# gpustack/llama-box

Measured on AMD Instinct MI355X. Metric: decode tokens/sec (batch-1) + prefill tok/s, Llama-3-8B Q4_K_M, higher is better.
Workload: dtype q4_K/q6_K weights x q8_K activations (int8 dot, f32 accumulate)

## Files before the change

llama_box_amd/csrc/backend.cpp:

```cpp
#include <dlfcn.h>

#include <algorithm>
#include <chrono>
#include <mutex>
#include <thread>

#include "common.h"
#include "kernels.h"

namespace mi355x {

int log_level() {
    static int lvl = [] {
        const char * e = getenv("GGML_MI355X_LOG");
        return e ? atoi(e) : 0;
    }();
    return lvl;
}

struct device_ctx {
    int device = 0;
    std::string name, description;
    ggml_backend_buffer_type buft{};
    ggml_backend_buffer_type buft_rowpar{};
// ... 163 lines not shown
        u->failed = true;
        return nullptr;
    }
    u->device = device;
    return u;
}
static void uploader_drain(int device) {
    if (device < 0 || device >= GGML_MI355X_MAX_DEVICES) return;
    uploader * u = &g_uploaders[device];
    if (u->device != device) return;
    std::lock_guard<std::mutex> lock(u->mtx);
    if (!u->in_flight) return;
    HIP_SOFT(hipStreamSynchronize(u->stream));
    for (bool & b : u->busy) b = false;
    u->in_flight = false;
}
static void uploader_join(int device, hipStream_t s) {
    if (device < 0 || device >= GGML_MI355X_MAX_DEVICES) return;
    uploader * u = &g_uploaders[device];
    if (u->device != device || !u->in_flight) return;
    std::lock_guard<std::mutex> lock(u->mtx);
    if (!u->in_flight) return;
    if (hipEventQuery(u->last) == hipSuccess) {
        for (bool & b : u->busy) b = false;
        u->in_flight = false;
        return;
    }
    (void) hipGetLastError();
    HIP_SOFT(hipStreamWaitEvent(s, u->last, 0));
}
// ... 255 lines not shown
static const char * be_get_name(ggml_backend_t be) { return ((backend_ctx *) be->context)->name.c_str(); }
static void be_free(ggml_backend_t be) {
    backend_ctx * c = (backend_ctx *) be->context;
    HIP_SOFT(hipSetDevice(c->device));
    HIP_SOFT(hipStreamSynchronize(c->stream));
    free_graph_cache(c);
    ip_free(c);
    tp_free(c);
    free_split_helpers(c);
    if (c->ws) HIP_NOTE(hipFree(c->ws));
    if (c->up_ring) HIP_NOTE(hipHostFree(c->up_ring));
    if (c->fa_lists) HIP_NOTE(hipFree(c->fa_lists));
    if (c->rope_tab) HIP_NOTE(hipFree(c->rope_tab));
    if (c->fa_arrive) HIP_NOTE(hipFree(c->fa_arrive));
    if (c->ss_buf) HIP_NOTE(hipFree(c->ss_buf));
    HIP_SOFT(hipStreamDestroy(c->stream));
    delete c;
    delete be;
}
void flush_uploads(backend_ctx * c) {
    if (c->up_pending.n == 0) return;
    launch_upload_multi(c->stream, c->up_pending);
    c->up_pending.n = 0;
}
static void be_set_tensor_async(ggml_backend_t be, ggml_tensor * t, const void * data, size_t offset, size_t size) {
    backend_ctx * c = (backend_ctx *) be->context;
    if (ip_any()) ip_host_access(t->view_src ? t->view_src->buffer : t->buffer, true);
    HIP_SOFT(hipSetDevice(c->device));
    note_mask_upload(t, data, offset, size);
    {
// ... 58 lines not shown
        HIP_SOFT(hipMemcpyAsync(dst->data, src->data, n, hipMemcpyDeviceToDevice, cs->stream));
    } else {
        HIP_SOFT(hipSetDevice(cs->device));
        HIP_SOFT(hipMemcpyPeerAsync(dst->data, cd->device, src->data, cs->device, n, cs->stream));
    }
    if (be_src != be_dst) {
        hipEvent_t ev;
        HIP_NOTE(hipEventCreateWithFlags(&ev, hipEventDisableTiming));
        HIP_SOFT(hipEventRecord(ev, cs->stream));
        HIP_SOFT(hipSetDevice(cd->device));
        HIP_SOFT(hipStreamWaitEvent(cd->stream, ev, 0));
        HIP_NOTE(hipEventDestroy(ev));
    }
    return true;
}
static void be_synchronize(ggml_backend_t be) {
    backend_ctx * c = (backend_ctx *) be->context;
    HIP_SOFT(hipSetDevice(c->device));
    flush_uploads(c);
    uploader_drain(c->device);
    HIP_SOFT(hipStreamSynchronize(c->stream));
}
static enum ggml_status be_graph_compute(ggml_backend_t be, ggml_cgraph * g) {
    backend_ctx * c = (backend_ctx *) be->context;
    if (hipSetDevice(c->device) != hipSuccess) return GGML_STATUS_FAILED;
    flush_uploads(c);
    uploader_join(c->device, c->stream);
    return graph_compute(c, g);
}
static void be_event_record(ggml_backend_t be, ggml_backend_event_t ev) {
    backend_ctx * c = (backend_ctx *) be->context;
    flush_uploads(c);
    HIP_SOFT(hipEventRecord((hipEvent_t) ev->context, c->stream));
}
static void be_event_wait(ggml_backend_t be, ggml_backend_event_t ev) {
// ... 180 lines not shown
    else if (k == "mmq_min_cols") c->opt.mmq_min_cols = v;
    else if (k == "mmq_i8") c->opt.mmq_i8 = v != 0;
    else if (k == "mm_merge") c->opt.mm_merge = v != 0;
    else if (k == "mmq_bn") c->opt.mmq_bn = v;
    else if (k == "mmq_skinny") c->opt.mmq_skinny = v != 0;
    else if (k == "skinny_rope") c->opt.skinny_rope = v != 0;
    else if (k == "skinny_mix") c->opt.skinny_mix = v != 0;
    else if (k == "softmax_mm") c->opt.softmax_mm = v != 0;
    else if (k == "attn_nf") c->opt.attn_nf = v != 0;
    else if (k == "fa_self_merge") c->opt.fa_self_merge = v != 0;
    else if (k == "ss_partials") c->opt.ss_partials = v != 0;
    else if (k == "tp_p2p") { if (!tp_p2p_enable(c, v != 0)) return -2; }
    else if (k == "tp_p2p_reset") { if (!tp_p2p_reset(c)) return -2; }
    else if (k == "fa_splits") c->opt.fa_splits = v;
    else if (k == "fa_wo") c->opt.fa_wo = v != 0;
    else if (k == "small_uploads") c->opt.small_uploads = v != 0;
    else if (k == "small_downloads") c->opt.small_downloads = v != 0;
    else if (k == "timing") c->opt.timing = v != 0;
    else if (k == "exec_update") c->opt.exec_update = v;
    else if (k == "shadow_capture") c->opt.shadow_capture = v;
    else if (k == "q80_min_cols") c->opt.q80_min_cols = v;
    else if (k == "decode_copy") c->opt.decode_copy = v != 0;
    else if (k == "decode_copy_headroom_gib") c->opt.decode_copy_headroom_gib = v;
    else if (k == "clear_failure") { if (v) clear_hip_failure(); }
    else if (k == "staged_upload") g_staged_upload.store(v != 0);
    else return -1;
    HIP_SOFT(hipStreamSynchronize(c->stream));
    free_graph_cache(c);
    return 0;
}
static int64_t api_get_stat(ggml_backend_t be, const char * key) {
    if (!be_is_ours(be)) return -1;
// ... 15 lines not shown
    if (k == "elided_conts") return c->st.elided_conts;
    if (k == "decode_copy_tensors") return c->st.decode_copy_tensors;
    if (k == "decode_copy_bytes") return c->st.decode_copy_bytes;
    if (k == "decode_copy_launches") return c->st.decode_copy_launches;
    if (k == "graph_exec_update_failures") return c->st.graph_exec_update_failures;
    if (k == "graph_evictions") return c->st.graph_evictions;
    if (k == "graph_cache_size") return (int64_t) c->graphs.size();
    if (k == "graph_launch_host_ns") return c->st.graph_launch_host_ns;
    if (k == "kernel_downloads") return c->st.kernel_downloads;
    if (k == "kv_image_nodes") return c->st.kv_image_nodes;
    if (k == "kv_native_nodes") return c->st.kv_native_nodes;
    if (k == "graph_key_host_ns") return c->st.graph_key_host_ns;
    if (k == "graph_compute_host_ns") return c->st.graph_compute_host_ns;
    if (k == "graph_key_fast_hits") return c->st.graph_key_fast_hits;
    if (k == "graph_key_collisions") return c->st.graph_key_collisions;
    if (k == "graph_early_captures") return c->st.graph_early_captures;
    if (k == "graph_shadow_captures") return c->st.graph_shadow_captures;
    if (k == "graph_capture_walk_ns") return c->st.graph_capture_walk_ns;
    if (k == "graph_exec_update_ns") return c->st.graph_exec_update_ns;
    if (k == "graph_shadow_eager_ns") return c->st.graph_shadow_eager_ns;
    if (k == "graph_exec_updates") return c->st.graph_exec_updates;
    if (k == "skinny_launches") return c->st.skinny_launches;
    if (k == "mmid_launches") return c->st.mmid_launches;
    if (k == "wide_launches") return c->st.wide_launches;
    if (k == "tiled_launches") return c->st.tiled_launches;
    if (k == "rope_epilogues") return c->st.rope_epilogues;
    if (k.rfind("ip_", 0) == 0) return ip_stat(c, key);
    if (k == "staged_upload_bytes") return (int64_t) g_uploaders[c->device].bytes;
    if (k == "staged_upload_us") return (int64_t) (g_uploaders[c->device].seconds * 1e6);
    return -1;
// ... 142 lines not shown
```

llama_box_amd/csrc/common.h:

```cpp
#pragma once
#include <hip/hip_runtime.h>
#include <hip/hip_ext.h>

#include <cstdint>
#include <cstdio>
#include <cstdlib>
#include <cstring>
#include <atomic>
#include <map>
#include <mutex>
#include <string>
#include <unordered_map>
#include <vector>

#include "../../include/ggml_mi355x.h"

#define MI_LOG(level, ...)                                    \
    do {                                                      \
        if ((level) <= mi355x::log_level()) {                 \
            fprintf(stderr, "ggml-mi355x: " __VA_ARGS__);     \
            fprintf(stderr, "\n");                            \
        }                                                     \
    } while (0)
#define MI_ERR(...) MI_LOG(0, __VA_ARGS__)
// ... 78 lines not shown
    bool qkv = true;
    int mmvq_max_cols = 2;
    int mmq_min_cols = 3;
    bool mmq_i8 = true;
    bool mm_merge = true;
    bool ss_partials = true;
    bool fa_self_merge = false;
    bool attn_nf = true;
    bool softmax_mm = true;
    bool skinny_rope = true;
    bool skinny_mix = true;
    bool mmq_skinny = true;
    int mmq_bn = 0;
    int fa_splits = 0;
    bool fa_wo = false;
    bool small_uploads = true;
    bool small_downloads = true;
    bool timing = false;
    int decode_copy_headroom_gib = 2;
    bool decode_copy = [] { const char * e = getenv("GGML_MI355X_DECODE_COPY"); return e ? atoi(e) != 0 : true; }();
    int exec_update = [] { const char * e = getenv("GGML_MI355X_EXEC_UPDATE"); return e ? atoi(e) : 1; }();
    int shadow_capture = [] { const char * e = getenv("GGML_MI355X_SHADOW_CAPTURE"); return e ? atoi(e) : 1; }();
    int q80_min_cols = [] { const char * e = getenv("GGML_MI355X_Q80_MIN_COLS"); return e ? atoi(e) : 33; }();
};

struct stats {
    int64_t graph_launches = 0, graph_captures = 0, eager_graphs = 0, kernel_launches = 0, fused_nodes = 0, allreduces = 0;
    int64_t p2p_allreduces = 0;
    int64_t ss_handoffs = 0;
    int64_t skinny_launches = 0;
    int64_t mmid_launches = 0;
    int64_t wide_launches = 0;
// ... 9 lines not shown
    int64_t kv_native_nodes = 0;
    int64_t kv_image_nodes = 0;
    int64_t kernel_downloads = 0;
    int64_t graph_early_captures = 0;
    int64_t graph_shadow_captures = 0;
    int64_t graph_capture_walk_ns = 0, graph_exec_update_ns = 0, graph_shadow_eager_ns = 0;
    int64_t graph_exec_updates = 0;
    int64_t decode_copy_tensors = 0;
    int64_t decode_copy_bytes = 0;
    int64_t decode_copy_launches = 0;
    int64_t elided_conts = 0;
    int64_t step_heads = 0;
    int64_t graph_exec_update_failures = 0;
    int64_t graph_evictions = 0;
    int64_t graph_key_collisions = 0;
};

struct tp_state;
struct split_helper;
struct ip_engine;

struct cached_graph {
    hipGraph_t graph = nullptr;
    hipGraphExec_t exec = nullptr;
    int seen = 0;
    uint64_t last_use = 0;
    int64_t allreduces = 0;
    int n_nodes = 0;
    int fa_form = 0;
    bool early_failed = false;
// ... 19 lines not shown
    uint64_t q8_epoch = 0;
    std::unordered_map<uint64_t, cached_graph> graphs;
    cached_graph * last_graph = nullptr;
    std::vector<uint64_t> key_scratch;
    uint64_t tick = 0;
    uint64_t decode_epoch = 0;
    bool capturing = false;
    bool mm_q5_major = false;
    tp_state * tp = nullptr;
    ip_engine * ip = nullptr;
    std::vector<split_helper *> split_helpers;
    hipEvent_t split_ready = nullptr;
    char * up_ring = nullptr;
    size_t up_cap = 0, up_head = 0;
    upload_batch up_pending{};
    double * ss_buf = nullptr;
    unsigned * fa_arrive = nullptr;
    static constexpr int fa_arrive_slots = 16384;
    float * rope_tab = nullptr;
    static constexpr int rope_tab_floats = 4096 * 256;
    int * fa_lists = nullptr;
    size_t fa_lists_bytes = 0;
    std::map<std::string, timing_slot> timing;
    std::vector<std::pair<std::string, std::pair<hipEvent_t, hipEvent_t>>> pending_events;
};

inline bool ensure_dyn_lds(const void * kernel, size_t bytes, std::atomic<uint32_t> & done) {
    int dev = 0;
    if (hipGetDevice(&dev) != hipSuccess || dev < 0 || dev >= 32) dev = 0;
    const uint32_t bit = 1u << dev;
// ... 98 lines not shown
```

llama_box_amd/csrc/graph.cpp:

```cpp
#include <algorithm>
#include <chrono>
#include <cmath>

#include "kernels.h"

namespace mi355x {

static bool is_kq23_type(int t) { return t == GGML_TYPE_Q2_K || t == GGML_TYPE_Q3_K; }
static bool is_quant(int t) { return t == GGML_TYPE_Q4_K || t == GGML_TYPE_Q5_K || t == GGML_TYPE_Q6_K || t == GGML_TYPE_Q8_0 || is_l32_type(t) || is_kq23_type(t); }
static bool l32_layout_ok(const ggml_tensor * a) {
    const size_t al = (a->type == GGML_TYPE_Q4_1 || a->type == GGML_TYPE_Q5_1 || a->type == GGML_TYPE_Q2_K) ? 4 : 2;
    if ((((uintptr_t) a->data) % al) || (a->nb[1] % al) || (a->nb[2] % al) || (a->nb[3] % al)) return false;
    return !buffer_is_rowpar(a->view_src ? a->view_src->buffer : a->buffer) && !buffer_is_split(a->buffer);
}
static inline int mmq_min_cols_for(const backend_ctx * c, int wtype) {
    if (is_kq23_type(wtype)) return 9;
    if (c->opt.mmq_min_cols != 3) return c->opt.mmq_min_cols;
    return (wtype == GGML_TYPE_Q4_K || (wtype == GGML_TYPE_Q6_K && !c->mm_q5_major)) ? 2 : 3;
}
static int act_kind(int wtype) {
    if (wtype == GGML_TYPE_Q4_1 || wtype == GGML_TYPE_Q5_1) return GGML_TYPE_Q8_1;
    return (wtype == GGML_TYPE_Q8_0 || is_l32_type(wtype)) ? GGML_TYPE_Q8_0 : GGML_TYPE_Q8_K;
}
static bool is_f32_contig(const ggml_tensor * t) { return t->type == GGML_TYPE_F32 && ggml_abi_is_contiguous(t); }
// ... 278 lines not shown
    const ggml_tensor * x;
    const ggml_tensor * w;
    float eps;
    const ggml_tensor * out;
};
struct exec_state {
    backend_ctx * c;
    ggml_cgraph * g;
    std::unordered_map<const ggml_tensor *, int> uses;
    mutable std::unordered_map<const ggml_tensor *, int> uses_global;
    size_t act_off = 0, aux_off = 0;
    std::unordered_map<const ggml_tensor *, deferred_norm> deferred;
    std::vector<char> done;
    std::vector<int> ooo;
    bool q8_fresh = false;
    const void * fa_list_mask = nullptr;
    int fa_list_tile = 0;
    struct { const ggml_tensor * b = nullptr; const ggml_tensor * fa = nullptr; const float * part = nullptr; int splits = 0; } fa_wo;
    const ggml_tensor * sk_dst = nullptr;
    splitk_src sk{};
    const ggml_tensor * epi_dst = nullptr;
    mmq_epi epi{};
    const void * rope_tab_pos = nullptr;
    const void * rope_tab_ff = nullptr;
    rope_params rope_tab_p{};
    int rope_tab_m = 0;
    int sk_next = -1;
    const ggml_tensor * ss_tensor = nullptr;
    int ss_n = 0;
    struct { int node = -1, n = 0, ks = 0, M = 0; mmq_mat_desc mats[3]; const ggml_tensor * dst[3]; const float * part = nullptr; } rs_sk;
// ... 79 lines not shown

static bool is_view_op(const ggml_tensor * t);
static bool ranges_overlap(const ggml_tensor * x, const ggml_tensor * y);
static bool quant_consumers_only(const exec_state & st, int at, const ggml_tensor * t);
static bool same_shape(const ggml_tensor * a, const ggml_tensor * b);
static bool run_mul_mat_q(exec_state & st, const ggml_tensor * w, const ggml_tensor * w2, const ggml_tensor * b, ggml_tensor * dst,
                          const ggml_tensor * add, const ggml_tensor * add2) {
    backend_ctx * c = st.c;
    const int64_t K = w->ne[0], N = w->ne[1];
    const int64_t M = b->ne[1] * b->ne[2] * b->ne[3];
    const double wbytes = (double) ggml_abi_row_size(w->type, K) * (double) N * (w2 ? 2.0 : 1.0);
    const bool kquant = is_kq23_type(w->type) || w->type == GGML_TYPE_Q4_K || w->type == GGML_TYPE_Q5_K || w->type == GGML_TYPE_Q6_K || (w->type == GGML_TYPE_Q8_0 && (K % 256) == 0);
    auto dn = st.deferred.find(b);
    const bool pro_norm = dn != st.deferred.end();
    const bool pro_fa = st.fa_wo.b == b && st.fa_wo.part != nullptr;
    static const bool dbg_no_pro_f32 = getenv("GGML_MI355X_DBG_NO_PRO_F32") != nullptr;
    const bool pro_f32 = !dbg_no_pro_f32 && !pro_norm && !pro_fa && c->opt.fusion && c->opt.prologue && kquant && M == 1 && b->type == GGML_TYPE_F32 && b->nb[0] == 4 && (((uintptr_t) b->data) & 15) == 0 &&
                         !ranges_overlap(dst, b);
    if (pro_fa && (w2 || pro_norm || !kquant || M != 1)) {
        MI_ERR("graph_compute: attention partials were left for a mat-vec that cannot merge them");
        return false;
    }
    if (pro_norm || pro_f32 || pro_fa) {
        mmvq_args a{};
        a.W = (const uint8_t *) w->data;
        a.W2 = w2 ? (const uint8_t *) w2->data : nullptr;
        a.Wp = decode_copy(c, w);
        a.W2p = w2 && a.Wp ? decode_copy(c, w2) : nullptr;
        if (w2 && !a.W2p) a.Wp = nullptr;
        c->st.decode_copy_launches += a.Wp != nullptr;
        a.w_nb1 = (int64_t) w->nb[1];
        a.type = w->type;
        a.K = (int) K;
        a.N = (int) N;
        a.ncols = 1;
        a.dst = (float *) dst->data;
        a.dst_stride = (int64_t) (dst->nb[1] / 4);
        a.add = add ? (const float *) add->data : nullptr;
        a.add2 = add2 ? (const float *) add2->data : nullptr;
        a.x = pro_norm ? (const float *) dn->second.x->data : (pro_fa ? nullptr : (const float *) b->data);
        if (pro_fa) {
            a.fa_part = st.fa_wo.part;
            a.fa_splits = st.fa_wo.splits;
            a.x_out = ranges_overlap(dst, st.fa_wo.fa) ? nullptr : (float *) st.fa_wo.fa->data;
            st.fa_wo.b = nullptr;
            st.fa_wo.part = nullptr;
        }
        a.norm_w = pro_norm ? (const float *) dn->second.w->data : nullptr;
        a.eps = pro_norm ? dn->second.eps : 0.0f;
        a.norm_out = (pro_norm && !ranges_overlap(dst, dn->second.out) && !ranges_overlap(dn->second.x, dn->second.out)) ? (float *) dn->second.out->data : nullptr;
        if (pro_norm && st.ss_tensor != nullptr && st.ss_tensor == dn->second.x) {
            a.ss_in = c->ss_buf;
            a.ss_n = st.ss_n;
            c->st.ss_handoffs++;
        }
        if (st.ss_tensor != nullptr && ranges_overlap(dst, st.ss_tensor)) st.ss_tensor = nullptr;
        if (c->opt.ss_partials && c->ss_buf != nullptr && (add || add2) && !w2 && !a.ss_in && launch_mmvq_ss_count(a) > 0) {
            a.ss_out = c->ss_buf;
            st.ss_tensor = dst;
            st.ss_n = launch_mmvq_ss_count(a);
        }
        char cls[64];
        snprintf(cls, sizeof(cls), "mmvq_%s%s_%s", type_tag(w->type), w2 ? "_glu" : "", pro_norm ? "normpro" : (pro_fa ? "attnpro" : "f32pro"));
        timed_scope ts(c, cls, wbytes, true);
        launch_mmvq(c->stream, a, 1);
        c->st.kernel_launches++;
        return true;
    }
    const int l32_form = (is_l32_type(w->type) && !w2 && !add2) ? mmq_l32_form(w->type, K, N, M) : 0;
    if (l32_form) {
        const bool one = act_kind(w->type) == GGML_TYPE_Q8_1;
        const void * act = quantized_src1(st, b, l32_form == 1 ? (one ? MI_ACT_Q81_PANEL : MI_ACT_Q80_PANEL) : w->type);
        timed_scope ts(c, (std::string("mmq_") + type_tag(w->type) + (l32_form == 1 ? "_skinny" : "")).c_str(), wbytes);
        const int64_t arows = add ? add->ne[1] * add->ne[2] * add->ne[3] : 0;
        launch_mmq_l32(c->stream, w->type, l32_form, (const uint8_t *) w->data, (int64_t) w->nb[1], (int) K, (int) N, (int) M, act, (float *) dst->data, (int64_t) (dst->nb[1] / 4),
                       add ? (const float *) add->data : nullptr, (!add || arows == 1) ? 0 : (int64_t) (add->nb[1] / 4));
        c->st.kernel_launches += l32_form == 1 ? (M + 31) / 32 : 1;
        c->st.skinny_launches += l32_form == 1;
// ... 1596 lines not shown
                    return 1;
                }
            }
            const ggml_tensor * q8_reader = nullptr;
            if (fuse && c->opt.prologue && a->ne[1] > 1 &&
                (a->ne[1] <= 128 || (p.n_splits >= 2 && fattn_combine_rows_applies((int) k->ne[0], a->ne[1], a->ne[2], a->ne[3], p.n_splits, n->src[4] ? (const float *) n->src[4]->data : nullptr))) &&
                use_count(st, n) == 1 && !(n->flags & GGML_TENSOR_FLAG_OUTPUT) && ggml_abi_is_contiguous(n)) {
                for (int k = i + 1; k < std::min(g->n_nodes, i + 4) && !q8_reader; ++k) {
                    const ggml_tensor * t = g->nodes[k];
                    if ((t->op == GGML_OP_RESHAPE || t->op == GGML_OP_VIEW) && t->src[0] == n && t->data == n->data && ggml_abi_is_contiguous(t) && t->ne[0] == n->ne[0] * n->ne[1] &&
                        t->ne[1] == n->ne[2] && quant_consumers_only(st, k, t) &&
                        fattn_q8_out_ok(qd, kd, m ? &md : nullptr, n->src[4] ? (const float *) n->src[4]->data : nullptr, TD(n), p))
                        q8_reader = t;
                }
            }
            if (q8_reader) p.q8_out = (char *) c->ws + st.act_off;
            g_fa_form = 0;
            launch_flash_attn(s, qd, kd, vd, m ? &md : nullptr, n->src[4] ? (const float *) n->src[4]->data : nullptr, TD(n), p, (char *) c->ws + st.aux_off);
            c->st.fa_form = g_fa_form;
            if (q8_reader) {
                mark_q8_cache(st, q8_reader);
                c->st.fused_nodes++;
            }
            c->st.kernel_launches += p.n_splits > 1 ? 2 : 1;
            return 1;
        }
        case GGML_OP_ARGMAX:
            launch_argmax(s, TD(a), TD(n));
            c->st.kernel_launches++;
            return 1;
        default:
            MI_ERR("graph_compute: unsupported op %d (node %d '%s')", (int) n->op, i, n->name);
            return -1;
    }
}

static bool run_nodes(backend_ctx * c, ggml_cgraph * g, const ws_plan & wp) {
// ... 29 lines not shown
        }
        st.q8_fresh = false;
        i += used;
    }
    return hipGetLastError() == hipSuccess;
}

static_assert(offsetof(ggml_tensor, ne) == offsetof(ggml_tensor, buffer) + 8 && offsetof(ggml_tensor, nb) == offsetof(ggml_tensor, ne) + 32 &&
              offsetof(ggml_tensor, op) == offsetof(ggml_tensor, nb) + 32 && offsetof(ggml_tensor, op_params) == offsetof(ggml_tensor, op) + 4 &&
              offsetof(ggml_tensor, flags) == offsetof(ggml_tensor, op_params) + 64 && offsetof(ggml_tensor, src) == offsetof(ggml_tensor, flags) + 4 &&
              offsetof(ggml_tensor, buffer) % 8 == 0 && offsetof(ggml_tensor, src) % 8 == 0,
              "graph key: {buffer, ne, nb, op, op_params, flags} must be one padding-free run of ggml_tensor");
static constexpr size_t KEY_NODE_RUN = (offsetof(ggml_tensor, src) - offsetof(ggml_tensor, buffer)) / 8;
static constexpr size_t KEY_SRC_RUN = (offsetof(ggml_tensor, op) - offsetof(ggml_tensor, buffer)) / 8;

template <class Put>
static inline bool walk_key(const ggml_cgraph * g, Put && put) {
    uint64_t w[2];
    w[0] = (uint64_t) (uint32_t) g->n_nodes;
    if (!put(w, 1)) return false;
    for (int i = 0; i < g->n_nodes; ++i) {
        const ggml_tensor * n = g->nodes[i];
        uint32_t present = 0;
        for (int s = 0; s < GGML_MAX_SRC; ++s) present |= n->src[s] ? 1u << s : 0u;
        const bool hinted = n->op == GGML_OP_FLASH_ATTN_EXT || n->op == GGML_OP_SOFT_MAX;
        w[0] = (uint64_t) (uint32_t) n->type | (uint64_t) present << 32 | (uint64_t) (hinted ? fa_mask_hint(n) : 0) << 48;
        w[1] = (uint64_t) (uintptr_t) n->data;
        if (!put(w, 2) || !put(&n->buffer, KEY_NODE_RUN)) return false;
        for (int s = 0; s < GGML_MAX_SRC; ++s) {
            const ggml_tensor * t = n->src[s];
            if (!t) continue;
            w[0] = (uint64_t) (uint32_t) t->type;
            w[1] = (uint64_t) (uintptr_t) t->data;
            if (!put(w, 2) || !put(&t->buffer, KEY_SRC_RUN)) return false;
        }
    }
    return true;
}
static bool key_equals(const ggml_cgraph * g, const std::vector<uint64_t> & key) {
    const uint64_t * at = key.data(), * const end = at + key.size();
    const bool same = walk_key(g, [&](const void * p, size_t n) {
        if ((size_t) (end - at) < n || memcmp(at, p, n * 8) != 0) return false;
        at += n;
        return true;
    });
    return same && at == end;
}
static void key_build(const ggml_cgraph * g, std::vector<uint64_t> & key) {
    key.clear();
    key.reserve((size_t) g->n_nodes * 48);
    walk_key(g, [&](const void * p, size_t n) {
        const size_t at = key.size();
        key.resize(at + n);
        memcpy(key.data() + at, p, n * 8);
        return true;
    });
}
bool graph_key_equals(const ggml_cgraph * g, const std::vector<uint64_t> & key) { return key_equals(g, key); }
void graph_key_build(const ggml_cgraph * g, std::vector<uint64_t> & key) { key_build(g, key); }
static uint64_t key_hash(const std::vector<uint64_t> & key) {
    uint64_t h[4] = {0x9E3779B97F4A7C15ull, 0xC2B2AE3D27D4EB4Full, 0x165667B19E3779F9ull, 0x27D4EB2F165667C5ull};
    auto fold = [](uint64_t a, uint64_t v) {
        const unsigned __int128 m = (unsigned __int128) (a ^ v) * 0xD6E8FEB86659FD93ull;
        return (uint64_t) m ^ (uint64_t) (m >> 64);
    };
    size_t i = 0;
    for (; i + 4 <= key.size(); i += 4)
        for (int l = 0; l < 4; ++l) h[l] = fold(h[l], key[i + l]);
    for (; i < key.size(); ++i) h[0] = fold(h[0], key[i]);
    return fold(fold(fold(h[0], h[1]), h[2]), h[3] ^ key.size());
}
// ... 204 lines not shown
```

llama_box_amd/csrc/kernels.h:

```cpp
#pragma once
#include "common.h"

namespace mi355x {

struct tdesc {
    char * data;
    int64_t ne[4];
    int64_t nb[4];
    int type;
};
inline tdesc TD(const ggml_tensor * t) {
    tdesc d;
    d.data = (char *) t->data;
    for (int i = 0; i < 4; ++i) {
        d.ne[i] = t->ne[i];
        d.nb[i] = (int64_t) t->nb[i];
    }
    d.type = (int) t->type;
    return d;
}

size_t quantized_act_bytes(int kind, int64_t K, int64_t rows);
void launch_quantize_act(hipStream_t s, int kind, const tdesc & src, void * dst);
#define MI_ACT_Q80_PANEL 1008
// ... 181 lines not shown
bool kv_store_type(int type);
bool kv_image_type(int type);
void launch_set_rows_kv(hipStream_t s, const tdesc & src, const tdesc & idx, const tdesc & dst);
void launch_set_rows_kv_pair(hipStream_t s, const tdesc & a0, const tdesc & i0, const tdesc & d0, const tdesc & a1, const tdesc & i1, const tdesc & d1);
void launch_cpy_kv(hipStream_t s, int type, const void * src, void * dst, int64_t n_values, bool to_type);
size_t kv_image_bytes(const tdesc & t);
tdesc kv_image_desc(const tdesc & t, void * image);
void launch_kv_images_f16(hipStream_t s, tdesc & k, tdesc & v, void * image);
void launch_argmax(hipStream_t s, const tdesc & src, const tdesc & dst);
#define MI_ARGSORT_MAX_COLS 1024
void launch_argsort(hipStream_t s, const tdesc & src, const tdesc & dst, int descending);
void launch_sum_rows(hipStream_t s, const tdesc & src, const tdesc & dst);
void launch_clamp(hipStream_t s, const tdesc & src, const tdesc & dst, float lo, float hi);
void launch_upload_multi(hipStream_t s, const upload_batch & b);
void launch_upload_small(hipStream_t s, void * dst, const void * pinned_src, size_t n);
void launch_copy2d(hipStream_t s, void * dst, size_t dpitch, const void * src, size_t spitch, size_t width, size_t height);
void launch_rebase_row_index(hipStream_t s, int64_t * dst, const int64_t * src, int64_t n_tok, int64_t full, int64_t ext, int64_t o0, int64_t n_ctx);
struct reduce_parts { const float * part[GGML_MI355X_MAX_DEVICES]; int n; };
void launch_reduce_parts(hipStream_t s, const reduce_parts & p, const float * add, float * dst, int64_t n);


struct rope_params {
    int n_dims, mode, n_ctx_orig;
    float freq_base, freq_scale, ext_factor, attn_factor, beta_fast, beta_slow;
    int sections[4];
};
void rope_host_consts(const rope_params & p, float & theta_scale, float & corr0, float & corr1);
void launch_rope_table(hipStream_t s, const int32_t * pos, const float * ff, const rope_params & p, int n_tok, float * tab);
void launch_step_head(hipStream_t s, const tdesc * a, const tdesc * idx, const tdesc * d, const float * cp_src, void * cp_dst, int64_t cp_n,
                      const int32_t * pos, const float * ff, const rope_params * p, int n_tok, float * tab);
// ... 111 lines not shown
```

llama_box_amd/csrc/mmvq.hip:

```cpp
#include <hip/hip_runtime.h>
#include <hip/hip_ext.h>

#include <algorithm>

#include <type_traits>

#include "mmvq_types.h"

namespace mi355x {

thread_local launch_probe g_launch_probe;


template <typename T, int NC, int R, bool GLU, int PRO, int WAVES>
__global__ void __launch_bounds__(WAVES * 64) k_mmvq(const mmvq_args a) {
    extern __shared__ __attribute__((aligned(16))) char smem[];
    typedef typename T::act act;
    constexpr int NT = WAVES * 64;
    const int tid = threadIdx.x, lane = tid & 63, wave = tid >> 6;
    const int nblk = a.K / T::BLK;
    const int npairs = nblk * T::PPB;
    const int row0 = (blockIdx.x * WAVES + wave) * R;

    const uint8_t * rows[R];
// ... 181 lines not shown
    const int nchk = a.K / 256;
    float4 v[4], g[4];
    double ssp[4] = {0.0, 0.0, 0.0, 0.0};
    item cur;
    float2 fml[PRO == 3 ? 16 : 1];
    float4 fr[PRO == 3 ? 12 : 1];
    if constexpr (PRO == 3) {
        const int S = a.fa_splits;
        const float * rec0 = a.fa_part + (size_t) (2 * min(wave, nchk - 1) + (lane >> 5)) * S * FA_REC;
#pragma unroll
        for (int sidx = 0; sidx < 16; ++sidx) fml[sidx] = *(const float2 *) (rec0 + (size_t) min(sidx, S - 1) * FA_REC + 128);
#pragma unroll
        for (int sidx = 0; sidx < 12; ++sidx) fr[sidx] = *(const float4 *) (rec0 + (size_t) min(sidx, S - 1) * FA_REC + 4 * (lane & 31));
        __builtin_amdgcn_sched_barrier(0);
    }
    if constexpr (PRO == 1 || PRO == 3) {
        if constexpr (PRO == 1) {
        const float4 * x4 = (const float4 *) a.x;
#pragma unroll
        for (int u = 0; u < 4; ++u) v[u] = x4[min(wave + u * WAVES, nchk - 1) * 64 + lane];
        __builtin_amdgcn_sched_barrier(0);
        }
        const int rc = min(row, a.N - 1);
        const uint8_t * rp = a.W + (size_t) rc * a.w_nb1;
        const uint8_t * rp2 = GLU ? a.W2 + (size_t) rc * a.w_nb1 : nullptr;
#pragma unroll
        for (int u = 0; u < U; ++u) {
            const int p = min(u * 64 + lane, npairs - 1);
            cur.w[u] = T::load(rp, p, nblk);
            if (GLU) cur.w2[u] = T::load(rp2, p, nblk);
        }
// ... 12 lines not shown
                if (b < nchk) {
                    v[u] = x4[b * 64 + lane];
                    g[u] = w4[b * 64 + lane];
                } else {
                    v[u] = make_float4(0.f, 0.f, 0.f, 0.f);
                    g[u] = v[u];
                }
            }
        }
    }

    if constexpr (PRO == 0) {
        const int nwords = (int) ((size_t) nblk * sizeof(act) / 4);
        const uint32_t * src = (const uint32_t *) a.act;
        uint32_t * dst = (uint32_t *) smem;
        if ((sizeof(act) & 15) == 0) {
            const int nvec = nwords >> 2;
            for (int i = tid; i < nvec; i += NT) ((uint4 *) dst)[i] = ((const uint4 *) src)[i];
        } else {
            for (int i = tid; i < nwords; i += NT) dst[i] = src[i];
        }
    } else if constexpr (PRO == 3) {
        act * yl = (act *) smem;
        const int S = a.fa_splits, hsel = lane >> 5, d0 = 4 * (lane & 31);
        constexpr float LOG2E = 1.4426950408889634f;
        for (int b0 = wave; b0 < nchk; b0 += WAVES) {
            const float * rec0 = a.fa_part + (size_t) (2 * b0 + hsel) * S * FA_REC;
            if (b0 != wave) {
#pragma unroll
                for (int sidx = 0; sidx < 16; ++sidx) fml[sidx] = *(const float2 *) (rec0 + (size_t) min(sidx, S - 1) * FA_REC + 128);
#pragma unroll
                for (int sidx = 0; sidx < 12; ++sidx) fr[sidx] = *(const float4 *) (rec0 + (size_t) min(sidx, S - 1) * FA_REC + d0);
            }
            float mn = -INFINITY;
#pragma unroll
// ... 231 lines not shown
        } else if (nc == 2) {
            if (glu) { if (fits) launch_one<T, 2, 1, true, 0, 4>(s, a, lds); else launch_one<T, 2, 1, true, 3, 4>(s, a, 0); }
            else     { if (fits) launch_one<T, 2, 1, false, 0, 4>(s, a, lds); else launch_one<T, 2, 1, false, 3, 4>(s, a, 0); }
        } else if (nc == 4) {
            if (glu) { if (fits) launch_one<T, 4, 1, true, 0, 4>(s, a, lds); else launch_one<T, 4, 1, true, 3, 4>(s, a, 0); }
            else     { if (fits) launch_one<T, 4, 1, false, 0, 4>(s, a, lds); else launch_one<T, 4, 1, false, 3, 4>(s, a, 0); }
        } else {
            if (glu) { if (fits) launch_one<T, 8, 1, true, 0, 4>(s, a, lds); else launch_one<T, 8, 1, true, 3, 4>(s, a, 0); }
            else     { if (fits) launch_one<T, 8, 1, false, 0, 4>(s, a, lds); else launch_one<T, 8, 1, false, 3, 4>(s, a, 0); }
        }
        done += nc;
    }
}

int launch_mmvq_ss_count(const mmvq_args & a) {
    if (a.ncols != 1 || a.W2 != nullptr || a.fa_part != nullptr || a.x == nullptr || (a.K % 256) != 0) return 0;
    return (int) std::min<int64_t>(256, ((int64_t) a.N + 15) / 16);
}

void launch_mmvq(hipStream_t s, const mmvq_args & a, int rows_per_wave) {
    switch (a.type) {
        case GGML_TYPE_Q2_K: launch_type<T_Q2K>(s, a, rows_per_wave); break;
        case GGML_TYPE_Q3_K: launch_type<T_Q3K>(s, a, rows_per_wave); break;
        case GGML_TYPE_Q4_K: launch_type<T_Q4K>(s, a, rows_per_wave); break;
        case GGML_TYPE_Q5_K: launch_type<T_Q5K>(s, a, rows_per_wave); break;
        case GGML_TYPE_Q6_K: launch_type<T_Q6K>(s, a, rows_per_wave); break;
        case GGML_TYPE_Q8_0: launch_type<T_Q80>(s, a, rows_per_wave); break;
        case GGML_TYPE_Q4_0: launch_type<T_Q40>(s, a, rows_per_wave); break;
        case GGML_TYPE_Q4_1: launch_type<T_Q41>(s, a, rows_per_wave); break;
        case GGML_TYPE_Q5_0: launch_type<T_Q50>(s, a, rows_per_wave); break;
        case GGML_TYPE_Q5_1: launch_type<T_Q51>(s, a, rows_per_wave); break;
// ... 9 lines not shown
```

llama_box_amd/csrc/ops.hip:

```cpp
#include <algorithm>

#include "dev_util.h"
#include "kernels.h"
#include "kv_dequant.h"

namespace mi355x {

__device__ __forceinline__ double block_sum_d(double v, double * sh) {
    v = wave_sum_d(v);
    const int lane = threadIdx.x & 63, wave = threadIdx.x >> 6;
    __syncthreads();
    if (lane == 0) sh[wave] = v;
    __syncthreads();
    double t = 0.0;
    const int nw = blockDim.x >> 6;
    for (int i = 0; i < nw; ++i) t += sh[i];
    return t;
}
__device__ __forceinline__ float block_max_f(float v, float * sh) {
    v = wave_max(v);
    const int lane = threadIdx.x & 63, wave = threadIdx.x >> 6;
    __syncthreads();
    if (lane == 0) sh[wave] = v;
    __syncthreads();
// ... 973 lines not shown
            if (i * 4 >= sg.n) break;
            ((uint32_t *) sg.dst)[i] = ((const uint32_t *) sg.src)[i];
        } else {
            if (i >= sg.n) break;
            sg.dst[i] = sg.src[i];
        }
    }
}
void launch_upload_multi(hipStream_t s, const upload_batch & b) {
    size_t most = 0;
    for (int i = 0; i < b.n; ++i) most = std::max(most, b.seg[i].n);
    const unsigned gx = (unsigned) std::min<size_t>(16, (most / 16 + 255) / 256 + 1);
    hipLaunchKernelGGL(k_upload_multi, dim3(gx, (unsigned) b.n), dim3(256), 0, s, b);
}

__global__ void __launch_bounds__(256) k_copy2d(char * __restrict__ dst, const size_t dpitch, const char * __restrict__ src, const size_t spitch, const size_t width, const int vec) {
    const size_t row = blockIdx.y;
    char * d = dst + row * dpitch;
    const char * s = src + row * spitch;
    for (size_t i = (size_t) blockIdx.x * 256 + threadIdx.x;; i += (size_t) gridDim.x * 256) {
        if (vec == 16) {
            if (i * 16 >= width) break;
            ((uint4 *) d)[i] = ((const uint4 *) s)[i];
        } else if (vec == 2) {
            if (i * 2 >= width) break;
            ((uint16_t *) d)[i] = ((const uint16_t *) s)[i];
        } else {
            if (i >= width) break;
            d[i] = s[i];
        }
// ... 105 lines not shown
```

llama_box_amd/csrc/tp_inproc.cpp:

```cpp
#include <algorithm>
#include <condition_variable>
#include <deque>
#include <list>
#include <mutex>
#include <thread>
#include <unordered_map>

#include "common.h"
#include "kernels.h"

namespace mi355x {

static constexpr int MAXD = GGML_MI355X_MAX_DEVICES;

struct sdesc {
    int kind = 0;
    int dim = 0;
    int64_t off[MAXD + 1] = {0};
};
static bool same_off(const sdesc & a, const sdesc & b, int n) {
    for (int i = 0; i <= n; ++i)
        if (a.off[i] != b.off[i]) return false;
    return true;
}
// ... 907 lines not shown
        for (int k = 0; k <= E->n_dev; ++k) o.off[k] = sd.off[k];
        o.stage_off = P->stage_bytes;
        int64_t widest = 0;
        for (int k = 0; k < E->n_dev; ++k) widest = std::max(widest, sd.off[k + 1] - sd.off[k]);
        P->stage_bytes += ((size_t) widest * (size_t) o.cols * 4 + 255) & ~(size_t) 255;
        P->outputs.push_back(o);
        for (int d = 0; d < E->n_dev; ++d) P->nodes[d][(size_t) i]->data = nullptr;
    }
    return P;
}

static bool same_options(const options & a, const options & b) {
    return a.graphs == b.graphs && a.fusion == b.fusion && a.prologue == b.prologue && a.qkv == b.qkv && a.mmvq_max_cols == b.mmvq_max_cols && a.mmq_min_cols == b.mmq_min_cols &&
           a.mmq_i8 == b.mmq_i8 && a.mm_merge == b.mm_merge && a.ss_partials == b.ss_partials && a.fa_self_merge == b.fa_self_merge && a.attn_nf == b.attn_nf &&
           a.softmax_mm == b.softmax_mm && a.skinny_rope == b.skinny_rope && a.skinny_mix == b.skinny_mix && a.mmq_skinny == b.mmq_skinny && a.mmq_bn == b.mmq_bn &&
           a.fa_splits == b.fa_splits && a.fa_wo == b.fa_wo && a.small_uploads == b.small_uploads && a.small_downloads == b.small_downloads && a.timing == b.timing;
}
static bool ensure_stage(ip_engine * E, size_t need) {
    if (need <= E->stage_size) return true;
    for (int d = 0; d < E->n_dev; ++d) {
        if (hipSetDevice(E->ordinal[d]) != hipSuccess) { (void) hipGetLastError(); return false; }
        (void) hipStreamSynchronize(E->ctx[d]->stream);
        if (E->stage[d]) (void) hipFree(E->stage[d]);
        E->stage[d] = nullptr;
        if (hipMalloc((void **) &E->stage[d], need + (1u << 20)) != hipSuccess) { (void) hipGetLastError(); (void) hipSetDevice(E->main->device); return false; }
        free_graph_cache(E->ctx[d]);
    }
    E->stage_size = need + (1u << 20);
    (void) hipSetDevice(E->main->device);
    return true;
}
// ... 210 lines not shown
```

Baseline: 589.2.

## Add poll-based sync, FA-to-Q8 matvec prologue, graph key node refs, act prefetch

```diff
diff --git a/llama_box_amd/csrc/backend.cpp b/llama_box_amd/csrc/backend.cpp
--- a/llama_box_amd/csrc/backend.cpp
+++ b/llama_box_amd/csrc/backend.cpp
@@ -1,4 +1,5 @@
 #include <dlfcn.h>
+#include <sched.h>
 
 #include <algorithm>
 #include <chrono>
@@ -201,6 +202,11 @@
     HIP_SOFT(hipStreamSynchronize(u->stream));
     for (bool & b : u->busy) b = false;
     u->in_flight = false;
+}
+static bool uploader_pending(int device) {
+    if (device < 0 || device >= GGML_MI355X_MAX_DEVICES) return false;
+    const uploader * u = &g_uploaders[device];
+    return u->device == device && u->in_flight;
 }
 static void uploader_join(int device, hipStream_t s) {
     if (device < 0 || device >= GGML_MI355X_MAX_DEVICES) return;
@@ -486,6 +492,7 @@
     if (c->rope_tab) HIP_NOTE(hipFree(c->rope_tab));
     if (c->fa_arrive) HIP_NOTE(hipFree(c->fa_arrive));
     if (c->ss_buf) HIP_NOTE(hipFree(c->ss_buf));
+    if (c->sync_word) HIP_NOTE(hipHostFree((void *) c->sync_word));
     HIP_SOFT(hipStreamDestroy(c->stream));
     delete c;
     delete be;
@@ -574,11 +581,44 @@
     }
     return true;
 }
+static bool poll_synchronize(backend_ctx * c) {
+    if (!c->sync_word) {
+        void * p = nullptr, * d = nullptr;
+        if (hipHostMalloc(&p, 64, hipHostMallocMapped) != hipSuccess || hipHostGetDevicePointer(&d, p, 0) != hipSuccess) {
+            (void) hipGetLastError();
+            if (p) (void) hipHostFree(p);
+            c->opt.poll_sync = false;
+            return false;
+        }
+        *(volatile uint32_t *) p = 0;
+        c->sync_word = (volatile uint32_t *) p;
+        c->sync_word_dev = (uint32_t *) d;
+    }
+    const uint32_t want = ++c->sync_epoch;
+    launch_epoch_store(c->stream, c->sync_word_dev, want);
+    if (hipGetLastError() != hipSuccess) return false;
+    auto now_ns = [] { return std::chrono::duration_cast<std::chrono::nanoseconds>(std::chrono::steady_clock::now().time_since_epoch()).count(); };
+    const int64_t t0 = now_ns(), prev = c->sync_prev_ns;
+    const int64_t tight_from = prev / 100 * 85, bound = std::max<int64_t>(2 * prev, 50 * 1000000ll);
+    bool seen = false;
+    for (;;) {
+        if (__atomic_load_n((const uint32_t *) c->sync_word, __ATOMIC_ACQUIRE) == want) { seen = true; break; }
+        const int64_t el = now_ns() - t0;
+        if (el > bound) break;
+        if (el + 200000 < tight_from) std::this_thread::sleep_for(std::chrono::microseconds(50));
+        else if (el < tight_from) sched_yield();
+    }
+    c->sync_prev_ns = now_ns() - t0;
+    c->st.sync_polls += seen;
+    return seen;
+}
 static void be_synchronize(ggml_backend_t be) {
     backend_ctx * c = (backend_ctx *) be->context;
     HIP_SOFT(hipSetDevice(c->device));
     flush_uploads(c);
+    const bool poll = c->opt.poll_sync && !ip_any() && !tp_active(c) && !uploader_pending(c->device);
     uploader_drain(c->device);
+    if (poll && poll_synchronize(c)) return;
     HIP_SOFT(hipStreamSynchronize(c->stream));
 }
 static enum ggml_status be_graph_compute(ggml_backend_t be, ggml_cgraph * g) {
@@ -789,8 +829,10 @@
     else if (k == "tp_p2p_reset") { if (!tp_p2p_reset(c)) return -2; }
     else if (k == "fa_splits") c->opt.fa_splits = v;
     else if (k == "fa_wo") c->opt.fa_wo = v != 0;
+    else if (k == "fa_q8_b1") c->opt.fa_q8_b1 = v != 0;
     else if (k == "small_uploads") c->opt.small_uploads = v != 0;
     else if (k == "small_downloads") c->opt.small_downloads = v != 0;
+    else if (k == "poll_sync") c->opt.poll_sync = v != 0;
     else if (k == "timing") c->opt.timing = v != 0;
     else if (k == "exec_update") c->opt.exec_update = v;
     else if (k == "shadow_capture") c->opt.shadow_capture = v;
@@ -836,6 +878,8 @@
     if (k == "graph_compute_host_ns") return c->st.graph_compute_host_ns;
     if (k == "graph_key_fast_hits") return c->st.graph_key_fast_hits;
     if (k == "graph_key_collisions") return c->st.graph_key_collisions;
+    if (k == "sync_polls") return c->st.sync_polls;
+    if (k == "fa_q8_b1_nodes") return c->st.fa_q8_b1_nodes;
     if (k == "graph_early_captures") return c->st.graph_early_captures;
     if (k == "graph_shadow_captures") return c->st.graph_shadow_captures;
     if (k == "graph_capture_walk_ns") return c->st.graph_capture_walk_ns;
diff --git a/llama_box_amd/csrc/common.h b/llama_box_amd/csrc/common.h
--- a/llama_box_amd/csrc/common.h
+++ b/llama_box_amd/csrc/common.h
@@ -116,8 +116,10 @@
     int mmq_bn = 0;
     int fa_splits = 0;
     bool fa_wo = false;
+    bool fa_q8_b1 = [] { const char * e = getenv("GGML_MI355X_FA_Q8_B1"); return e ? atoi(e) != 0 : false; }();
     bool small_uploads = true;
     bool small_downloads = true;
+    bool poll_sync = [] { const char * e = getenv("GGML_MI355X_POLL_SYNC"); return e ? atoi(e) != 0 : false; }();
     bool timing = false;
     int decode_copy_headroom_gib = 2;
     bool decode_copy = [] { const char * e = getenv("GGML_MI355X_DECODE_COPY"); return e ? atoi(e) != 0 : true; }();
@@ -157,6 +159,8 @@
     int64_t graph_exec_update_failures = 0;
     int64_t graph_evictions = 0;
     int64_t graph_key_collisions = 0;
+    int64_t fa_q8_b1_nodes = 0;
+    int64_t sync_polls = 0;
 };
 
 struct tp_state;
@@ -206,6 +210,10 @@
     char * up_ring = nullptr;
     size_t up_cap = 0, up_head = 0;
     upload_batch up_pending{};
+    volatile uint32_t * sync_word = nullptr;
+    uint32_t * sync_word_dev = nullptr;
+    uint32_t sync_epoch = 0;
+    int64_t sync_prev_ns = 0;
     double * ss_buf = nullptr;
     unsigned * fa_arrive = nullptr;
     static constexpr int fa_arrive_slots = 16384;
diff --git a/llama_box_amd/csrc/graph.cpp b/llama_box_amd/csrc/graph.cpp
--- a/llama_box_amd/csrc/graph.cpp
+++ b/llama_box_amd/csrc/graph.cpp
@@ -316,6 +316,7 @@
     std::vector<char> done;
     std::vector<int> ooo;
     bool q8_fresh = false;
+    const ggml_tensor * q8_b1 = nullptr;
     const void * fa_list_mask = nullptr;
     int fa_list_tile = 0;
     struct { const ggml_tensor * b = nullptr; const ggml_tensor * fa = nullptr; const float * part = nullptr; int splits = 0; } fa_wo;
@@ -425,14 +426,22 @@
     auto dn = st.deferred.find(b);
     const bool pro_norm = dn != st.deferred.end();
     const bool pro_fa = st.fa_wo.b == b && st.fa_wo.part != nullptr;
+    const bool pro_q8 = st.q8_b1 != nullptr && st.q8_b1 == b;
+    if (pro_q8) {
+        st.q8_b1 = nullptr;
+        if (w2 || pro_norm || pro_fa || M != 1 || act_kind(w->type) != GGML_TYPE_Q8_K || c->q8_src != b->data || c->q8_kind != GGML_TYPE_Q8_K || c->q8_bytes != ggml_abi_nbytes(b)) {
+            MI_ERR("graph_compute: Q8_K blocks were left for a mat-vec that cannot read them");
+            return false;
+        }
+    }
     static const bool dbg_no_pro_f32 = getenv("GGML_MI355X_DBG_NO_PRO_F32") != nullptr;
-    const bool pro_f32 = !dbg_no_pro_f32 && !pro_norm && !pro_fa && c->opt.fusion && c->opt.prologue && kquant && M == 1 && b->type == GGML_TYPE_F32 && b->nb[0] == 4 && (((uintptr_t) b->data) & 15) == 0 &&
+    const bool pro_f32 = !dbg_no_pro_f32 && !pro_norm && !pro_fa && !pro_q8 && c->opt.fusion && c->opt.prologue && kquant && M == 1 && b->type == GGML_TYPE_F32 && b->nb[0] == 4 && (((uintptr_t) b->data) & 15) == 0 &&
                          !ranges_overlap(dst, b);
     if (pro_fa && (w2 || pro_norm || !kquant || M != 1)) {
         MI_ERR("graph_compute: attention partials were left for a mat-vec that cannot merge them");
         return false;
     }
-    if (pro_norm || pro_f32 || pro_fa) {
+    if (pro_norm || pro_f32 || pro_fa || pro_q8) {
         mmvq_args a{};
         a.W = (const uint8_t *) w->data;
         a.W2 = w2 ? (const uint8_t *) w2->data : nullptr;
@@ -449,7 +458,8 @@
         a.dst_stride = (int64_t) (dst->nb[1] / 4);
         a.add = add ? (const float *) add->data : nullptr;
         a.add2 = add2 ? (const float *) add2->data : nullptr;
-        a.x = pro_norm ? (const float *) dn->second.x->data : (pro_fa ? nullptr : (const float *) b->data);
+        a.x = pro_norm ? (const float *) dn->second.x->data : ((pro_fa || pro_q8) ? nullptr : (const float *) b->data);
+        if (pro_q8) a.act = (const char *) c->ws + st.act_off;
         if (pro_fa) {
             a.fa_part = st.fa_wo.part;
             a.fa_splits = st.fa_wo.splits;
@@ -472,7 +482,7 @@
             st.ss_n = launch_mmvq_ss_count(a);
         }
         char cls[64];
-        snprintf(cls, sizeof(cls), "mmvq_%s%s_%s", type_tag(w->type), w2 ? "_glu" : "", pro_norm ? "normpro" : (pro_fa ? "attnpro" : "f32pro"));
+        snprintf(cls, sizeof(cls), "mmvq_%s%s_%s", type_tag(w->type), w2 ? "_glu" : "", pro_norm ? "normpro" : (pro_fa ? "attnpro" : (pro_q8 ? "q8pro" : "f32pro")));
         timed_scope ts(c, cls, wbytes, true);
         launch_mmvq(c->stream, a, 1);
         c->st.kernel_launches++;
@@ -2099,6 +2109,26 @@
                         q8_reader = t;
                 }
             }
+            bool q8_b1 = false;
+            if (!q8_reader && fuse && c->opt.prologue && c->opt.fa_q8_b1 && !p.arrive && a->ne[1] == 1 && a->ne[3] == 1 && (a->ne[2] % 2) == 0 && use_count(st, n) == 1 &&
+                !(n->flags & GGML_TENSOR_FLAG_OUTPUT) && ggml_abi_is_contiguous(n)) {
+                for (int k = i + 1; k < std::min(g->n_nodes, i + 4) && !q8_reader; ++k) {
+                    const ggml_tensor * t = g->nodes[k];
+                    if (!((t->op == GGML_OP_RESHAPE || t->op == GGML_OP_VIEW) && t->src[0] == n && t->data == n->data && ggml_abi_is_contiguous(t) && t->ne[0] == n->ne[0] * n->ne[1] &&
+                          t->ne[1] == n->ne[2] && use_count(st, t) == 1 && quant_consumers_only(st, k, t)))
+                        continue;
+                    const ggml_tensor * mm = nullptr;
+                    for (int j = k + 1; j < g->n_nodes && !mm; ++j)
+                        if (g->nodes[j]->src[1] == t) mm = g->nodes[j];
+                    const ggml_tensor * w = mm ? mm->src[0] : nullptr;
+                    if (w && (w->ne[0] % 256) == 0 && w->ne[0] == t->ne[0] && w->ne[2] == 1 && w->ne[3] == 1 && rows_contig(w) && quant_mm_ok(mm) && mm->type == GGML_TYPE_F32 &&
+                        !(tp_active(c) && buffer_is_rowpar(w->view_src ? w->view_src->buffer : w->buffer)) &&
+                        fattn_q8_out_ok(qd, kd, m ? &md : nullptr, n->src[4] ? (const float *) n->src[4]->data : nullptr, TD(n), p)) {
+                        q8_reader = t;
+                        q8_b1 = true;
+                    }
+                }
+            }
             if (q8_reader) p.q8_out = (char *) c->ws + st.act_off;
             g_fa_form = 0;
             launch_flash_attn(s, qd, kd, vd, m ? &md : nullptr, n->src[4] ? (const float *) n->src[4]->data : nullptr, TD(n), p, (char *) c->ws + st.aux_off);
@@ -2106,6 +2136,10 @@
             if (q8_reader) {
                 mark_q8_cache(st, q8_reader);
                 c->st.fused_nodes++;
+            }
+            if (q8_b1) {
+                st.q8_b1 = q8_reader;
+                c->st.fa_q8_b1_nodes++;
             }
             c->st.kernel_launches += p.n_splits > 1 ? 2 : 1;
             return 1;
@@ -2165,47 +2199,78 @@
 static constexpr size_t KEY_NODE_RUN = (offsetof(ggml_tensor, src) - offsetof(ggml_tensor, buffer)) / 8;
 static constexpr size_t KEY_SRC_RUN = (offsetof(ggml_tensor, op) - offsetof(ggml_tensor, buffer)) / 8;
 
-template <class Put>
-static inline bool walk_key(const ggml_cgraph * g, Put && put) {
+static constexpr uint64_t KEY_SRC_NODE = 1ull << 63;
+static constexpr size_t KEY_SRC_SLOT = 2 + KEY_SRC_RUN;
+static inline bool key_src_may_be_node(const ggml_tensor * t) { return t->op != GGML_OP_NONE || (t->flags & GGML_TENSOR_FLAG_PARAM) != 0; }
+static inline void key_node_head(const ggml_tensor * n, uint64_t w[2]) {
+    uint32_t present = 0;
+    for (int s = 0; s < GGML_MAX_SRC; ++s) present |= n->src[s] ? 1u << s : 0u;
+    const bool hinted = n->op == GGML_OP_FLASH_ATTN_EXT || n->op == GGML_OP_SOFT_MAX;
+    w[0] = (uint64_t) (uint32_t) n->type | (uint64_t) present << 32 | (uint64_t) (hinted ? fa_mask_hint(n) : 0) << 48;
+    w[1] = (uint64_t) (uintptr_t) n->data;
+}
+static bool key_equals(const ggml_cgraph * g, const std::vector<uint64_t> & key) {
+    const uint64_t * at = key.data(), * const end = at + key.size();
+    if (at == end || *at++ != (uint64_t) (uint32_t) g->n_nodes) return false;
     uint64_t w[2];
-    w[0] = (uint64_t) (uint32_t) g->n_nodes;
-    if (!put(w, 1)) return false;
     for (int i = 0; i < g->n_nodes; ++i) {
         const ggml_tensor * n = g->nodes[i];
-        uint32_t present = 0;
-        for (int s = 0; s < GGML_MAX_SRC; ++s) present |= n->src[s] ? 1u << s : 0u;
-        const bool hinted = n->op == GGML_OP_FLASH_ATTN_EXT || n->op == GGML_OP_SOFT_MAX;
-        w[0] = (uint64_t) (uint32_t) n->type | (uint64_t) present << 32 | (uint64_t) (hinted ? fa_mask_hint(n) : 0) << 48;
-        w[1] = (uint64_t) (uintptr_t) n->data;
-        if (!put(w, 2) || !put(&n->buffer, KEY_NODE_RUN)) return false;
+        if ((size_t) (end - at) < 2 + KEY_NODE_RUN) return false;
+        key_node_head(n, w);
+        if (at[0] != w[0] || at[1] != w[1] || memcmp(at + 2, &n->buffer, KEY_NODE_RUN * 8) != 0) return false;
+        at += 2 + KEY_NODE_RUN;
         for (int s = 0; s < GGML_MAX_SRC; ++s) {
             const ggml_tensor * t = n->src[s];
             if (!t) continue;
-            w[0] = (uint64_t) (uint32_t) t->type;
-            w[1] = (uint64_t) (uintptr_t) t->data;
-            if (!put(w, 2) || !put(&t->buffer, KEY_SRC_RUN)) return false;
-        }
-    }
-    return true;
-}
-static bool key_equals(const ggml_cgraph * g, const std::vector<uint64_t> & key) {
-    const uint64_t * at = key.data(), * const end = at + key.size();
-    const bool same = walk_key(g, [&](const void * p, size_t n) {
-        if ((size_t) (end - at) < n || memcmp(at, p, n * 8) != 0) return false;
-        at += n;
-        return true;
-    });
-    return same && at == end;
+            if ((size_t) (end - at) < KEY_SRC_SLOT) return false;
+            if (at[0] & KEY_SRC_NODE) {
+                const uint64_t j = at[0] & ~KEY_SRC_NODE;
+                if (j >= (uint64_t) i || g->nodes[j] != t || !key_src_may_be_node(t)) return false;
+            } else {
+                if (key_src_may_be_node(t))
+                    for (int j = 0; j < i; ++j)
+                        if (g->nodes[j] == t) return false;
+                if (at[0] != (uint64_t) (uint32_t) t->type || at[1] != (uint64_t) (uintptr_t) t->data || memcmp(at + 2, &t->buffer, KEY_SRC_RUN * 8) != 0) return false;
+            }
+            at += KEY_SRC_SLOT;
+        }
+    }
+    return at == end;
 }
 static void key_build(const ggml_cgraph * g, std::vector<uint64_t> & key) {
     key.clear();
     key.reserve((size_t) g->n_nodes * 48);
-    walk_key(g, [&](const void * p, size_t n) {
+    auto put = [&](const void * p, size_t n) {
         const size_t at = key.size();
         key.resize(at + n);
         memcpy(key.data() + at, p, n * 8);
-        return true;
-    });
+    };
+    std::unordered_map<const ggml_tensor *, int> index;
+    index.reserve((size_t) g->n_nodes * 2);
+    uint64_t w[2];
+    w[0] = (uint64_t) (uint32_t) g->n_nodes;
+    put(w, 1);
+    for (int i = 0; i < g->n_nodes; ++i) {
+        const ggml_tensor * n = g->nodes[i];
+        key_node_head(n, w);
+        put(w, 2);
+        put(&n->buffer, KEY_NODE_RUN);
+        for (int s = 0; s < GGML_MAX_SRC; ++s) {
+            const ggml_tensor * t = n->src[s];
+            if (!t) continue;
+            const auto it = key_src_may_be_node(t) ? index.find(t) : index.end();
+            if (it != index.end()) {
+                const uint64_t slot[KEY_SRC_SLOT] = {KEY_SRC_NODE | (uint64_t) it->second};
+                put(slot, KEY_SRC_SLOT);
+            } else {
+                w[0] = (uint64_t) (uint32_t) t->type;
+                w[1] = (uint64_t) (uintptr_t) t->data;
+                put(w, 2);
+                put(&t->buffer, KEY_SRC_RUN);
+            }
+        }
+        index.emplace(n, i);
+    }
 }
 bool graph_key_equals(const ggml_cgraph * g, const std::vector<uint64_t> & key) { return key_equals(g, key); }
 void graph_key_build(const ggml_cgraph * g, std::vector<uint64_t> & key) { key_build(g, key); }
diff --git a/llama_box_amd/csrc/kernels.h b/llama_box_amd/csrc/kernels.h
--- a/llama_box_amd/csrc/kernels.h
+++ b/llama_box_amd/csrc/kernels.h
@@ -219,6 +219,7 @@
 void launch_clamp(hipStream_t s, const tdesc & src, const tdesc & dst, float lo, float hi);
 void launch_upload_multi(hipStream_t s, const upload_batch & b);
 void launch_upload_small(hipStream_t s, void * dst, const void * pinned_src, size_t n);
+void launch_epoch_store(hipStream_t s, uint32_t * mapped, uint32_t v);
 void launch_copy2d(hipStream_t s, void * dst, size_t dpitch, const void * src, size_t spitch, size_t width, size_t height);
 void launch_rebase_row_index(hipStream_t s, int64_t * dst, const int64_t * src, int64_t n_tok, int64_t full, int64_t ext, int64_t o0, int64_t n_ctx);
 struct reduce_parts { const float * part[GGML_MI355X_MAX_DEVICES]; int n; };
diff --git a/llama_box_amd/csrc/mmvq.hip b/llama_box_amd/csrc/mmvq.hip
--- a/llama_box_amd/csrc/mmvq.hip
+++ b/llama_box_amd/csrc/mmvq.hip
@@ -219,7 +219,20 @@
         for (int sidx = 0; sidx < 12; ++sidx) fr[sidx] = *(const float4 *) (rec0 + (size_t) min(sidx, S - 1) * FA_REC + 4 * (lane & 31));
         __builtin_amdgcn_sched_barrier(0);
     }
-    if constexpr (PRO == 1 || PRO == 3) {
+    constexpr bool ACT16 = (sizeof(act) & 15) == 0;
+    uint4 ya = make_uint4(0u, 0u, 0u, 0u);
+    uint32_t yw[2] = {0u, 0u};
+    if constexpr (PRO == 0) {
+        const int nwords = (int) ((size_t) nblk * sizeof(act) / 4);
+        if constexpr (ACT16) {
+            ya = ((const uint4 *) a.act)[min(tid, (nwords >> 2) - 1)];
+        } else {
+            yw[0] = ((const uint32_t *) a.act)[min(tid, nwords - 1)];
+            yw[1] = ((const uint32_t *) a.act)[min(tid + NT, nwords - 1)];
+        }
+        __builtin_amdgcn_sched_barrier(0);
+    }
+    if constexpr (PRO == 0 || PRO == 1 || PRO == 3) {
         if constexpr (PRO == 1) {
         const float4 * x4 = (const float4 *) a.x;
 #pragma unroll
@@ -262,11 +275,14 @@
         const int nwords = (int) ((size_t) nblk * sizeof(act) / 4);
         const uint32_t * src = (const uint32_t *) a.act;
         uint32_t * dst = (uint32_t *) smem;
-        if ((sizeof(act) & 15) == 0) {
+        if constexpr (ACT16) {
             const int nvec = nwords >> 2;
-            for (int i = tid; i < nvec; i += NT) ((uint4 *) dst)[i] = ((const uint4 *) src)[i];
+            if (tid < nvec) ((uint4 *) dst)[tid] = ya;
+            for (int i = tid + NT; i < nvec; i += NT) ((uint4 *) dst)[i] = ((const uint4 *) src)[i];
         } else {
-            for (int i = tid; i < nwords; i += NT) dst[i] = src[i];
+            if (tid < nwords) dst[tid] = yw[0];
+            if (tid + NT < nwords) dst[tid + NT] = yw[1];
+            for (int i = tid + 2 * NT; i < nwords; i += NT) dst[i] = src[i];
         }
     } else if constexpr (PRO == 3) {
         act * yl = (act *) smem;
@@ -528,7 +544,8 @@
 }
 
 int launch_mmvq_ss_count(const mmvq_args & a) {
-    if (a.ncols != 1 || a.W2 != nullptr || a.fa_part != nullptr || a.x == nullptr || (a.K % 256) != 0) return 0;
+    if (a.ncols != 1 || a.W2 != nullptr || a.fa_part != nullptr || (a.K % 256) != 0) return 0;
+    if (a.x == nullptr && !(a.act != nullptr && (a.type == GGML_TYPE_Q2_K || a.type == GGML_TYPE_Q3_K || a.type == GGML_TYPE_Q4_K || a.type == GGML_TYPE_Q5_K || a.type == GGML_TYPE_Q6_K) && (size_t) (a.K / 256) * sizeof(q8k_dev) <= 60 * 1024)) return 0;
     return (int) std::min<int64_t>(256, ((int64_t) a.N + 15) / 16);
 }
 
diff --git a/llama_box_amd/csrc/ops.hip b/llama_box_amd/csrc/ops.hip
--- a/llama_box_amd/csrc/ops.hip
+++ b/llama_box_amd/csrc/ops.hip
@@ -1011,6 +1011,11 @@
     hipLaunchKernelGGL(k_upload_multi, dim3(gx, (unsigned) b.n), dim3(256), 0, s, b);
 }
 
+__global__ void __launch_bounds__(64) k_epoch_store(uint32_t * p, const uint32_t v) {
+    if (threadIdx.x == 0) __hip_atomic_store(p, v, __ATOMIC_RELEASE, __HIP_MEMORY_SCOPE_SYSTEM);
+}
+void launch_epoch_store(hipStream_t s, uint32_t * mapped, uint32_t v) { hipLaunchKernelGGL(k_epoch_store, dim3(1), dim3(64), 0, s, mapped, v); }
+
 __global__ void __launch_bounds__(256) k_copy2d(char * __restrict__ dst, const size_t dpitch, const char * __restrict__ src, const size_t spitch, const size_t width, const int vec) {
     const size_t row = blockIdx.y;
     char * d = dst + row * dpitch;
diff --git a/llama_box_amd/csrc/tp_inproc.cpp b/llama_box_amd/csrc/tp_inproc.cpp
--- a/llama_box_amd/csrc/tp_inproc.cpp
+++ b/llama_box_amd/csrc/tp_inproc.cpp
@@ -945,7 +945,7 @@
     return a.graphs == b.graphs && a.fusion == b.fusion && a.prologue == b.prologue && a.qkv == b.qkv && a.mmvq_max_cols == b.mmvq_max_cols && a.mmq_min_cols == b.mmq_min_cols &&
            a.mmq_i8 == b.mmq_i8 && a.mm_merge == b.mm_merge && a.ss_partials == b.ss_partials && a.fa_self_merge == b.fa_self_merge && a.attn_nf == b.attn_nf &&
            a.softmax_mm == b.softmax_mm && a.skinny_rope == b.skinny_rope && a.skinny_mix == b.skinny_mix && a.mmq_skinny == b.mmq_skinny && a.mmq_bn == b.mmq_bn &&
-           a.fa_splits == b.fa_splits && a.fa_wo == b.fa_wo && a.small_uploads == b.small_uploads && a.small_downloads == b.small_downloads && a.timing == b.timing;
+           a.fa_splits == b.fa_splits && a.fa_wo == b.fa_wo && a.fa_q8_b1 == b.fa_q8_b1 && a.small_uploads == b.small_uploads && a.small_downloads == b.small_downloads && a.timing == b.timing;
 }
 static bool ensure_stage(ip_engine * E, size_t need) {
     if (need <= E->stage_size) return true;
```

After: 590.0 (median of 2 runs). Within noise of the previous version (+0.1%).
